# lastz/lastz

Hardware: AMD Instinct MI355X
Metric: Gbp-of-target aligned/sec (whole job, --nogapped HSP path, both strands) (higher is better)
Workload: dtype s32

## Files before the change

lastz_amd/csrc/lz_lut.hpp:

```cpp
#pragma once
#include "lz_common.hpp"

#define LZ_PAD2         128
#define LZ_LUT_ENTRIES  4096
#define LZ_LUT_TOTAL    (2 * LZ_LUT_ENTRIES)
#define LZ_LUT_WIN_G    15
#define LZ_LUT_WIN_B    60
#define LZ_LUT_MAXWIN   3
#define LZ_GRAY(c)      ((c) ^ ((c) >> 1))

struct alignas(8) LzLutEntry { u32 ab; u32 sc; };

struct LzLutParams {
    const u8* t2; const u8* q2;
    const u8* tsp; const u8* qsp;
    const u8* t2x; const u8* tspx;
    const u8* tcode; const u8* qcode;
    s32 xdrop;
};

struct LzLutScan { u32 s; s32 run, best; u32 room, used, alive, nwin; };

#if defined(__HIP_DEVICE_COMPILE__)
LZ_HD u32 lz_alignbit(u32 hi, u32 lo, u32 sh) { return __builtin_amdgcn_alignbit(hi, lo, sh); }
LZ_HD s32 lz_sdot4(u32 a, s32 acc) { return __builtin_amdgcn_sdot4((int)a, 0x01010101, acc, false); }
LZ_HD s32 lz_sdot4m(u32 a, u32 ones, s32 acc) { return __builtin_amdgcn_sdot4((int)a, (int)ones, acc, false); }
LZ_HD u32 lz_byte_pair(u32 hi_src, u32 lo_src, int k)
{ return __builtin_amdgcn_perm(hi_src, lo_src, 0x0C0C0000u | ((u32)(4 + k) << 8) | (u32)k); }
#define LZ_UNROLL_ALL _Pragma("unroll")
#else
LZ_HD u32 lz_alignbit(u32 hi, u32 lo, u32 sh) { sh &= 31u; return sh ? (lo >> sh) | (hi << (32u - sh)) : lo; }
LZ_HD s32 lz_sdot4(u32 a, s32 acc) { for (int k = 0; k < 4; k++) acc += (s32)(int8_t)(a >> (8 * k)); return acc; }
LZ_HD s32 lz_sdot4m(u32 a, u32 ones, s32 acc) { for (int k = 0; k < 4; k++) acc += (s32)(int8_t)(a >> (8 * k)) * (s32)((ones >> (8 * k)) & 0xFFu); return acc; }
LZ_HD u32 lz_byte_pair(u32 hi_src, u32 lo_src, int k) { return (((hi_src >> (8 * k)) & 0xFFu) << 8) | ((lo_src >> (8 * k)) & 0xFFu); }
#define LZ_UNROLL_ALL
#endif
LZ_HD u32 lz_ctz64(u64 x) { return (u32)__builtin_ctzll(x); }
LZ_HD u32 lz_clz64(u64 x) { return (u32)__builtin_clzll(x); }

template <bool SPECIAL> struct LzLutRaw { LzVec16 tv, qv, tm, qm; };
template <> struct LzLutRaw<false> { LzVec16 tv, qv; };
#define LZ_LUT_GBYTE(RIGHT_, g_) ((RIGHT_) ? (g_) : 14 - (g_))
template <bool RIGHT, bool SPECIAL>
LZ_HD void lz_lut_fetch(const LzLutParams& P, u32 s_, s32 diag, LzLutRaw<SPECIAL>& raw)
{
    const u32 st = RIGHT ? s_ + (u32)LZ_PAD2 : s_ - 1u + (u32)LZ_PAD2;
    const u32 sq = st - (u32)diag;
    const u32 back = RIGHT ? 0u : 15u;
    raw.tv = lz_load16(P.t2 + ((st >> 2) - back)); raw.qv = lz_load16(P.q2 + ((sq >> 2) - back));
    if constexpr (SPECIAL) {
        const u32 mback = RIGHT ? 0u : 14u;
        raw.tm = lz_load16(P.tsp + ((st >> 3) - mback)); raw.qm = lz_load16(P.qsp + ((sq >> 3) - mback));
    }
}
template <bool RIGHT>
LZ_HD u64 lz_lut_mask64(const LzVec16& v, s64 s)
{
    if (RIGHT) {
        const u32 k = (u32)((u64)(s + LZ_PAD2) & 7u);
        return ((u64)lz_alignbit(v.w[2], v.w[1], k) << 32) | lz_alignbit(v.w[1], v.w[0], k);
    }
    const u32 k = 17u + (u32)((u64)(s - 1 + LZ_PAD2) & 7u);
    return ((u64)lz_alignbit(v.w[3], v.w[2], k) << 32) | lz_alignbit(v.w[2], v.w[1], k);
}

template <bool RIGHT, bool SPECIAL, bool LIMCHK>
LZ_HD void lz_lut_window(const LzLutParams& P, const LzLutEntry* lut, s32 diag, LzLutScan& st, const LzLutRaw<SPECIAL>& raw, const s32* ctab = nullptr)
{
    const s32 X = P.xdrop;
    const LzLutEntry* const tab = lut + (RIGHT ? 0 : LZ_LUT_ENTRIES);
    const u32 spad = RIGHT ? st.s + (u32)LZ_PAD2 : st.s - 1u + (u32)LZ_PAD2, qpad = spad - (u32)diag;
    u32 tw[4], qw[4];
    {
        const u32 a = RIGHT ? 2u * (spad & 3u) : 2u * (spad & 3u) + 2u;
        const u32 b = RIGHT ? 2u * (qpad & 3u) : 2u * (qpad & 3u) + 2u;
        tw[0] = lz_alignbit(raw.tv.w[1], raw.tv.w[0], a); tw[1] = lz_alignbit(raw.tv.w[2], raw.tv.w[1], a); tw[2] = lz_alignbit(raw.tv.w[3], raw.tv.w[2], a); tw[3] = raw.tv.w[3] >> a;
        qw[0] = lz_alignbit(raw.qv.w[1], raw.qv.w[0], b); qw[1] = lz_alignbit(raw.qv.w[2], raw.qv.w[1], b); qw[2] = lz_alignbit(raw.qv.w[3], raw.qv.w[2], b); qw[3] = raw.qv.w[3] >> b;
    }
    u32 lim = st.room < (u32)LZ_LUT_WIN_B ? st.room : (u32)LZ_LUT_WIN_B;
    bool soft = false;
    if constexpr (SPECIAL) {
        const s64 s = (s64)st.s, sq = s - (s64)diag;
        const u64 sm = lz_lut_mask64<RIGHT>(raw.tm, s) | lz_lut_mask64<RIGHT>(raw.qm, sq);
        const u32 nsp = sm ? (RIGHT ? lz_ctz64(sm) : lz_clz64(sm)) : 64u;
        if (nsp < lim) { soft = true; lim = nsp; }
    }
    u32 xw[4], wc[4];
    LZ_UNROLL_ALL
    for (int k = 0; k < 4; k++) {
        xw[k] = tw[k] ^ qw[k];
        const u32 u = (tw[k] & 0x11111111u) | ((tw[k] >> 1) & 0x22222222u);
        wc[k] = (u | (u >> 2)) & 0x0F0F0F0Fu;
    }
    const u32 glim = lim >> 2;
    s32 run = st.run, m = run - st.best + X;
    u32 np = 0, fsc = 0;
#if !defined(LZ_LUT_NO_EARLY_EXIT) && defined(__HIP_DEVICE_COMPILE__)
    {
#define LZ_LUT_ENTRY_OF(g_) tab[lz_byte_pair(wc[LZ_LUT_GBYTE(RIGHT, g_) >> 2], xw[LZ_LUT_GBYTE(RIGHT, g_) >> 2], LZ_LUT_GBYTE(RIGHT, g_) & 3)]
        LzLutEntry ea = LZ_LUT_ENTRY_OF(0), eb = ea;
        LZ_UNROLL_ALL
        for (int g = 0; g < LZ_LUT_WIN_G; g += 2) {
            if (g + 1 < LZ_LUT_WIN_G) eb = LZ_LUT_ENTRY_OF(g + 1);
            if (m < (s32)(ea.ab & 0xFFFFu)) goto groups_done;
            if (LIMCHK && (u32)g >= glim) goto groups_done;
            { const s32 bq = (s32)ea.ab >> 16; m = lz_sdot4(ea.sc, m < bq ? m : bq); run = lz_sdot4(ea.sc, run); np = (u32)g + 1u; }
            if (g + 1 < LZ_LUT_WIN_G) {
                if (g + 2 < LZ_LUT_WIN_G) ea = LZ_LUT_ENTRY_OF(g + 2);
                if (m < (s32)(eb.ab & 0xFFFFu)) goto groups_done;
                if (LIMCHK && (u32)(g + 1) >= glim) goto groups_done;
                { const s32 bq = (s32)eb.ab >> 16; m = lz_sdot4(eb.sc, m < bq ? m : bq); run = lz_sdot4(eb.sc, run); np = (u32)g + 2u; }
            }
        }
        groups_done:
        fsc = (np & 1u) ? eb.sc : ea.sc;
#undef LZ_LUT_ENTRY_OF
    }
#else
    {
        bool dead = false;
        LZ_UNROLL_ALL
        for (int g = 0; g < LZ_LUT_WIN_G; g++) {
            const int by = LZ_LUT_GBYTE(RIGHT, g);
            const LzLutEntry e = tab[lz_byte_pair(wc[by >> 2], xw[by >> 2], by & 3)];
            if (!dead) fsc = e.sc;
            dead = dead | (m < (s32)(e.ab & 0xFFFFu));
            if (LIMCHK) dead = dead | ((u32)g >= glim);
            const s32 bq = (s32)e.ab >> 16;
            const s32 t = lz_sdot4(e.sc, m < bq ? m : bq);
            const s32 r2 = lz_sdot4(e.sc, run);
            m = dead ? m : t; run = dead ? run : r2; np += dead ? 0u : 1u;
        }
    }
#endif
    u32 r = 0;
    if (np < (u32)LZ_LUT_WIN_G) { r = lim - 4u * np; if (r > 4u) r = 4u; }
    s32 best = run - m + X;
    const u32 sc = fsc;
    bool stop = false; u32 j = 0;
    if (LIMCHK) {
        LZ_UNROLL_ALL
        for (u32 b = 0; b < 4; b++) {
            const bool on = !stop && b < r;
            const s32 nr = run + (s32)(int8_t)(sc >> (8u * b));
            run = on ? nr : run;
            j += on ? 1u : 0u;
            best = (on && nr > best) ? nr : best;
            stop = stop | (on && nr < best - X);
        }
    } else if (r) {
        const s32 p1 = lz_sdot4m(sc, 0x00000001u, m), p2 = lz_sdot4m(sc, 0x00000101u, m), p3 = lz_sdot4m(sc, 0x00010101u, m), p4 = lz_sdot4(sc, m);
        const s32 q2 = p1 | p2, q3 = q2 | p3;
        j = 4u + (u32)(p1 >> 31) + (u32)(q2 >> 31) + (u32)(q3 >> 31);
        stop = (q3 | p4) < 0;
    }
    st.run = run; st.best = best;
    st.used += 4u * np + j;
    st.nwin++;
    if (stop) st.alive = 0;
    else if (r == 4u) st.alive = 2;
    else if (soft) {
        if constexpr (SPECIAL) {
            const u32 p1 = RIGHT ? st.s + lim : st.s - 1u - lim;
            const s32 v = ctab[(LZ_CODE_CLASS(P.tcode[(s64)p1]) << 5) | LZ_CODE_CLASS(P.qcode[(s64)p1 - (s64)diag])];
            st.run += v; st.used += 1u;
            if (st.run > st.best) st.best = st.run;
            const u32 eaten = lim + 1u;
            if (st.run < st.best - X || eaten == st.room) st.alive = 0;
            else { st.alive = 1; st.room -= eaten; st.s = RIGHT ? st.s + eaten : st.s - eaten; }
        }
    }
    else if (lim == st.room) st.alive = 0;
    else { st.alive = 1; st.room -= (u32)LZ_LUT_WIN_B; st.s = RIGHT ? st.s + (u32)LZ_LUT_WIN_B : st.s - (u32)LZ_LUT_WIN_B; }
}
template <bool SPECIAL, bool LIMCHK>
LZ_HD void lz_lut_window_pair(const LzLutParams& P, const LzLutEntry* lut, s32 diag, LzLutScan& L, LzLutScan& R,
                              const LzLutRaw<SPECIAL>& rawl, const LzLutRaw<SPECIAL>& rawr, bool do_l, bool do_r, const s32* ctab = nullptr)
{
    if (do_l) lz_lut_window<false, SPECIAL, LIMCHK>(P, lut, diag, L, rawl, ctab);
    if (do_r) lz_lut_window<true, SPECIAL, LIMCHK>(P, lut, diag, R, rawr, ctab);
}
template <bool RIGHT, bool SPECIAL>
LZ_HD void lz_lut_step(const LzLutParams& P, const LzLutEntry* lut, s32 diag, LzLutScan& st, const s32* ctab = nullptr)
{
    LzLutRaw<SPECIAL> raw;
    lz_lut_fetch<RIGHT, SPECIAL>(P, st.s, diag, raw);
    if (!SPECIAL && st.room >= (u32)LZ_LUT_WIN_B) lz_lut_window<RIGHT, SPECIAL, false>(P, lut, diag, st, raw);
    else                                           lz_lut_window<RIGHT, SPECIAL, true>(P, lut, diag, st, raw, ctab);
}

LZ_HD void lz_lut_init(u64 key, u32 tlen, u32 qlen, s32& diag, LzLutScan& L, LzLutScan& R)
{
    const u32 pos2 = (u32)key;
    diag = (s32)(u32)(key >> 32);
    const u32 pos1 = pos2 + (u32)diag;
    const s32 stopl = diag > 0 ? diag : 0;
    const s32 stopr = ((s32)tlen <= (s32)qlen + diag) ? (s32)tlen : (s32)qlen + diag;
    L.s = R.s = pos1; L.run = L.best = R.run = R.best = 0; L.used = R.used = 0; L.nwin = R.nwin = 0;
    L.room = (u32)((s32)pos1 - stopl); R.room = (u32)(stopr - (s32)pos1);
    L.alive = ((s32)pos1 > stopl) ? 1u : 0u; R.alive = ((s32)pos1 < stopr) ? 1u : 0u;
}

LZ_HD u32 lz_lut_summary(const LzLutScan& L, const LzLutScan& R, s32 min_score)
{
    u32 summ = (L.used & 0xFFu) | ((R.used & 0xFFu) << 8);
    if (L.alive || R.alive || L.best + R.best >= min_score) summ |= LZ_SUMM_SLOW;
    return summ;
}

template <bool SPECIAL>
LZ_HD u32 lz_lut_probe_hit(const LzLutParams& P, const LzLutEntry* lut, u32 tlen, u32 qlen, s32 min_score, u64 key, const s32* ctab = nullptr)
{
    s32 diag; LzLutScan L, R;
    lz_lut_init(key, tlen, qlen, diag, L, R);
    while (L.alive == 1 && L.nwin < (u32)LZ_LUT_MAXWIN) lz_lut_step<false, SPECIAL>(P, lut, diag, L, ctab);
    while (R.alive == 1 && R.nwin < (u32)LZ_LUT_MAXWIN) lz_lut_step<true, SPECIAL>(P, lut, diag, R, ctab);
    return lz_lut_summary(L, R, min_score);
}

LZ_HD u64 lz_hit_record(u64 key, u32 summ)
{
    const u32 pos2 = (u32)key, diag = (u32)(key >> 32);
    const bool slow = (summ & LZ_SUMM_SLOW) != 0;
    const u64 payload = slow ? (u64)(diag >> 16) : (u64)(summ & 0xFFFFu);
    return (u64)pos2 | ((u64)(diag & 0xFFu) << 31) | (payload << 39) | (slow ? (1ull << 63) : 0ull);
}
#define LZ_REC_TAG(r)     ((u32)((r) >> 55) & 0xFFu)
#define LZ_REC_UNTAG(r)   ((r) & ~(0xFFull << 55))
LZ_HD u64 lz_hit_record_tagged(u64 key, u32 summ) { return lz_hit_record(key, summ) | ((u64)((u32)(key >> 40) & 0xFFu) << 55); }

#define LZ_WCTX_BYTES 32
struct alignas(16) LzWctx { u32 w[LZ_WCTX_BYTES / 4]; };
LZ_HD u32 lz_wctx_first_byte(u32 pos1) { return ((pos1 - 1u + (u32)LZ_PAD2) >> 2) - 15u; }
LZ_HD u32 lz_wctx_right_offset(u32 pos1) { return ((pos1 + (u32)LZ_PAD2) >> 2) - lz_wctx_first_byte(pos1); }
LZ_HD LzWctx lz_wctx_make(const u8* two, u32 pos1) { LzWctx e; __builtin_memcpy(&e, two + lz_wctx_first_byte(pos1), LZ_WCTX_BYTES); return e; }
LZ_HD void lz_wctx_windows(const LzWctx& e, u32 pos1, LzVec16& tl, LzVec16& tr)
{
    const bool at16 = lz_wctx_right_offset(pos1) == 16u;
    LZ_UNROLL_ALL
    for (int k = 0; k < 4; k++) {
        tl.w[k] = e.w[k];
        const u32 at15 = lz_alignbit(e.w[4 + k], e.w[3 + k], 24u);
        tr.w[k] = at16 ? e.w[4 + k] : at15;
    }
}

#define LZ_REC_POS2(r)    ((u32)((r) & 0x7FFFFFFFu))
#define LZ_REC_LOW8(r)    ((u32)((r) >> 31) & 0xFFu)
#define LZ_REC_PAYLOAD(r) ((u32)((r) >> 39) & 0xFFFFu)
#define LZ_REC_SLOW(r)    ((u32)((r) >> 63))
LZ_HD u64 lz_rec_with_index(u64 r, u32 idx)
{ return (r & ~((0xFFull << 31) | (0x1Full << 55))) | ((u64)(idx & 0xFFu) << 31) | ((u64)((idx >> 8) & 0x1Fu) << 55); }
#define LZ_REC_INDEX(r)   (((u32)((r) >> 31) & 0xFFu) | (((u32)((r) >> 55) & 0x1Fu) << 8))

template <class Emit>
LZ_HD void lz_settle_record(const LzExtendParams& P, const s32* score_tab, u64 rec, u32 h ,
                            u32& dend, u64& n_ext, u64& n_bp, Emit&& emit)
{
    const u32 p2 = LZ_REC_POS2(rec);
    if (dend > p2 - P.seed_len) return;
    n_ext++;
    const u32 pay = LZ_REC_PAYLOAD(rec);
    if (!LZ_REC_SLOW(rec)) {
        const u32 room = p2 - dend, dlo = pay & 0xFFu, dext = pay >> 8;
        const u32 extent = p2 + dext;
        n_bp += (dlo < room ? dlo : room) + dext;
        if (extent > dend) dend = extent;
        return;
    }
    const s32 diag = (s32)((pay << 16) | h);
    dend = lz_reextend(P, score_tab, p2, diag, dend, n_bp, emit);
}
```

lastz_amd/csrc/scan_kernels.hip:

```cpp
#include <hip/hip_runtime.h>
#include <algorithm>
#include <type_traits>
#include "lz_ctx.hpp"
#include "lz_host.hpp"
#include "lz_lut.hpp"
#include "lz_seed_dev.hpp"

#define LZ_SC_ROUNDS 4

struct LzScanTask { u32 idx; s32 diag; LzLutScan L, R; };
static_assert(sizeof(LzScanTask) == 64, "LzScanTask: one 64-byte line per task");
#define LZ_SC_TPB 512
template <int MODE> struct LzScanShared {
    union {
        LzLutEntry lut[LZ_LUT_TOTAL];
        struct { s32 tab[LZ_NCLASS * LZ_NCLASS]; s32 tab8[64]; } bc;
    };
    s32 ctab[MODE == 1 ? LZ_NCLASS * LZ_NCLASS : 1];
};

template <bool SP>
__device__ __forceinline__ void lz_scan_round(const LzExtendParams& P, const LzLutParams& Q, const LzLutEntry* lut, const s32* ctab, u64 key, bool valid,
                                              const LzLutRaw<SP>& rawl, const LzLutRaw<SP>& rawr, u32 idx, u32 lane,
                                              u32& summ_out, LzScanTask* __restrict__ my_tasks, u32& my_n, u32 region_cap)
{
    constexpr bool HLIM = SP;
    s32 diag; LzLutScan L, R;
    lz_lut_init(key, P.tlen, P.qlen, diag, L, R);
    if (!valid) { L.alive = 0; R.alive = 0; }
    const bool ql = L.alive && !HLIM && L.room < (u32)LZ_LUT_WIN_B, qr = R.alive && !HLIM && R.room < (u32)LZ_LUT_WIN_B;
    lz_lut_window_pair<SP, HLIM>(Q, lut, diag, L, R, rawl, rawr, L.alive && !ql, R.alive && !qr, ctab);
    const bool more = valid && (L.alive == 1 || R.alive == 1);
    const u64 mm = __ballot(more);
    bool queued = false;
    if (mm) {
        const u32 slot = my_n + (u32)__popcll(mm & ((1ull << lane) - 1ull));
        if (more && slot < region_cap) {
            LzScanTask t; t.idx = idx; t.diag = diag; t.L = L; t.R = R;
            my_tasks[slot] = t; queued = true;
        }
        my_n += (u32)__popcll(mm);
    }
    summ_out = queued ? 0u : lz_lut_summary(L, R, P.min_score);
}
template <bool SP>
__device__ __forceinline__ void lz_scan_fetch(const LzLutParams& Q, u64 key, LzLutRaw<SP>& rawl, LzLutRaw<SP>& rawr)
{
    const u32 pos2 = (u32)key, pos1 = pos2 + (u32)(key >> 32);
    const s32 diag = (s32)(u32)(key >> 32);
    const u32 stl = pos1 - 1u + (u32)LZ_PAD2, str = pos1 + (u32)LZ_PAD2;
    const u32 bl = (stl >> 2) - 15u, br = str >> 2;
    const u32 ol = bl + (bl & ~31u);
    rawl.tv = lz_load16(Q.t2x + ol); rawr.tv = lz_load16(Q.t2x + (ol + (br - bl)));
    const u32 sql = stl - (u32)diag, sqr = str - (u32)diag;
    rawl.qv = lz_load16(Q.q2 + ((sql >> 2) - 15u)); rawr.qv = lz_load16(Q.q2 + (sqr >> 2));
    if constexpr (SP) {
        const u32 ml = (stl >> 3) - 14u, mr = str >> 3;
        const u32 oml = ml + (ml & ~31u);
        rawl.tm = lz_load16(Q.tspx + oml); rawr.tm = lz_load16(Q.tspx + (oml + (mr - ml)));
        rawl.qm = lz_load16(Q.qsp + ((sql >> 3) - 14u)); rawr.qm = lz_load16(Q.qsp + (sqr >> 3));
    }
}

template <int MODE, int TPB, int WPE>
__global__ void __launch_bounds__(TPB, WPE)
k_scan_hits(LzExtendParams P, LzLutParams Q, const u64* __restrict__ keys, u64 n,
            const s32* __restrict__ score_tab_g, const LzLutEntry* __restrict__ lut_g,
            u32* __restrict__ summ, u8* __restrict__ bins, LzScanTask* __restrict__ tasks, u32* __restrict__ n_tasks, u32 region_cap)
{
    __shared__ LzScanShared<MODE> sh;
    const u32 tid = threadIdx.x, lane = tid & 63u, w = tid >> 6;
    if (MODE == 1) { for (u32 k = tid; k < LZ_NCLASS * LZ_NCLASS; k += TPB) sh.ctab[k] = score_tab_g[k]; }
    if (MODE < 2) { for (u32 k = tid; k < LZ_LUT_TOTAL; k += TPB) sh.lut[k] = lut_g[k]; }
    else {
        for (u32 k = tid; k < LZ_NCLASS * LZ_NCLASS; k += TPB) sh.bc.tab[k] = score_tab_g[k];
        if (tid < 64) sh.bc.tab8[tid] = score_tab_g[(tid >> 3) * LZ_NCLASS + (tid & 7)];
    }
    __syncthreads();
    const LzLutEntry* lut = sh.lut;
    const s32* const ctab = sh.ctab;
    constexpr bool SP = MODE == 1;
    constexpr u32 SPAN = 64u * LZ_SC_ROUNDS;
    static_assert(LZ_SC_ROUNDS == 4, "the round pipeline below is written out for four rounds per span");
    const u64 nspans = (n + SPAN - 1) / SPAN, wstride = (u64)gridDim.x * (TPB / 64);
    const u32 region = blockIdx.x * (TPB / 64) + w;
    LzScanTask* const my_tasks = tasks + (size_t)region * region_cap;
    u32 my_n = 0;
    u64 span = (u64)blockIdx.x * (TPB / 64) + w;
    if (MODE == 2) {
        for (; span < nspans; span += wstride) {
            const u64 base = span * SPAN;
            const u32 span_n = (n - base < (u64)SPAN) ? (u32)(n - base) : SPAN;
#pragma unroll 1
            for (u32 r = 0; r < LZ_SC_ROUNDS; r++) {
                const u32 li = r * 64u + lane;
                if (li < span_n) { const u64 kk = keys[base + li]; summ[base + li] = lz_probe_hit(P, sh.bc.tab, sh.bc.tab8, P.cls8 != 0, kk); bins[base + li] = (u8)LZ_KEY_BIN(kk); }
            }
        }
    } else if (span < nspans) {
        typedef u64 lz_u64x2 __attribute__((ext_vector_type(2)));
        auto load_keys = [&](u64 sp, u64& a0, u64& a1, u64& a2, u64& a3) {
            const u64 base = sp * SPAN;
            const u32 sn = (n - base < (u64)SPAN) ? (u32)(n - base) : SPAN;
            const u32 l4 = 4u * lane;
            const u64* kp = keys + base + l4;
            if (l4 + 3u < sn) {
                const lz_u64x2 x = LZ_NT_LD(reinterpret_cast<const lz_u64x2*>(kp)), y = LZ_NT_LD(reinterpret_cast<const lz_u64x2*>(kp + 2));
                a0 = x.x; a1 = x.y; a2 = y.x; a3 = y.y;
            } else {
                a0 = (l4 < sn) ? LZ_NT_LD(kp) : 0ull;           a1 = (l4 + 1u < sn) ? LZ_NT_LD(kp + 1) : 0ull;
                a2 = (l4 + 2u < sn) ? LZ_NT_LD(kp + 2) : 0ull;  a3 = 0ull;
            }
        };
        u64 k0, k1, k2, k3;
        load_keys(span, k0, k1, k2, k3);
        LzLutRaw<SP> al, ar, bl, br;
        lz_scan_fetch<SP>(Q, k0, al, ar);
#pragma unroll 1
        for (;;) {
            const u64 base = span * SPAN;
            const u32 span_n = (n - base < (u64)SPAN) ? (u32)(n - base) : SPAN;
            const u32 l4 = 4u * lane;
            const u32 ib = (u32)base + l4;
            const bool more_spans = span + wstride < nspans;
            u64 n0 = 0, n1 = 0, n2 = 0, n3 = 0;
            u32 s0, s1, s2, s3;
            lz_scan_fetch<SP>(Q, k1, bl, br);
            lz_scan_round<SP>(P, Q, lut, ctab, k0, l4 < span_n, al, ar, ib, lane, s0, my_tasks, my_n, region_cap);
            if (more_spans) load_keys(span + wstride, n0, n1, n2, n3);
            lz_scan_fetch<SP>(Q, k2, al, ar);
            lz_scan_round<SP>(P, Q, lut, ctab, k1, l4 + 1u < span_n, bl, br, ib + 1u, lane, s1, my_tasks, my_n, region_cap);
            lz_scan_fetch<SP>(Q, k3, bl, br);
            lz_scan_round<SP>(P, Q, lut, ctab, k2, l4 + 2u < span_n, al, ar, ib + 2u, lane, s2, my_tasks, my_n, region_cap);
            if (more_spans) lz_scan_fetch<SP>(Q, n0, al, ar);
            lz_scan_round<SP>(P, Q, lut, ctab, k3, l4 + 3u < span_n, bl, br, ib + 3u, lane, s3, my_tasks, my_n, region_cap);
            const u32 pbytes = LZ_KEY_BIN(k0) | (LZ_KEY_BIN(k1) << 8) | (LZ_KEY_BIN(k2) << 16) | (LZ_KEY_BIN(k3) << 24);
            if (l4 + 3u < span_n) {
                typedef u32 lz_u32x4 __attribute__((ext_vector_type(4)));
                lz_u32x4 sv4; sv4.x = s0; sv4.y = s1; sv4.z = s2; sv4.w = s3;
                LZ_NT_ST(sv4, reinterpret_cast<lz_u32x4*>(summ + ib));
                LZ_NT_ST(pbytes, reinterpret_cast<u32*>(bins + ib));
            } else {
                if (l4 < span_n)      { summ[ib] = s0;      bins[ib] = (u8)pbytes; }
                if (l4 + 1u < span_n) { summ[ib + 1u] = s1; bins[ib + 1u] = (u8)(pbytes >> 8); }
                if (l4 + 2u < span_n) { summ[ib + 2u] = s2; bins[ib + 2u] = (u8)(pbytes >> 16); }
            }
            if (!more_spans) break;
            span += wstride; k0 = n0; k1 = n1; k2 = n2; k3 = n3;
        }
    }
    if (lane == 0) n_tasks[region] = my_n < region_cap ? my_n : region_cap;
}

#define LZ_ST_TPB 512
template <int MODE, bool TAGGED>
__global__ void __launch_bounds__(LZ_ST_TPB)
k_scan_tasks(LzExtendParams P, LzLutParams Q, const LzLutEntry* __restrict__ lut_g, const s32* __restrict__ score_tab_g, const LzScanTask* __restrict__ tasks,
             const u32* __restrict__ n_tasks, u32 n_regions, u32 region_cap, std::conditional_t<TAGGED, u64, u32>* __restrict__ out)
{
    constexpr bool SP = MODE == 1;
    static_assert(!(SP && TAGGED), "pos1 is recovered from the windows a scan ran: without special bytes only");
    __shared__ LzLutEntry lut[LZ_LUT_TOTAL];
    __shared__ s32 ctab[SP ? LZ_NCLASS * LZ_NCLASS : 1];
    for (u32 k = threadIdx.x; k < LZ_LUT_TOTAL; k += LZ_ST_TPB) lut[k] = lut_g[k];
    if (SP) for (u32 k = threadIdx.x; k < LZ_NCLASS * LZ_NCLASS; k += LZ_ST_TPB) ctab[k] = score_tab_g[k];
    __syncthreads();
    for (u32 region = blockIdx.x; region < n_regions; region += gridDim.x) {
        const u32 nt = n_tasks[region];
        for (u32 k = threadIdx.x; k < nt; k += (u32)LZ_ST_TPB) {
            const LzScanTask t = tasks[(size_t)region * region_cap + k];
            LzLutScan L = t.L, R = t.R;
            u32 pos1 = 0;
            if constexpr (TAGGED) pos1 = L.alive == 1 ? L.s + (u32)LZ_LUT_WIN_B * L.nwin : R.s - (u32)LZ_LUT_WIN_B * R.nwin;
            while (L.alive == 1 && L.nwin < (u32)LZ_LUT_MAXWIN) lz_lut_step<false, SP>(Q, lut, t.diag, L, ctab);
            while (R.alive == 1 && R.nwin < (u32)LZ_LUT_MAXWIN) lz_lut_step<true, SP>(Q, lut, t.diag, R, ctab);
            const u32 summ = lz_lut_summary(L, R, P.min_score);
            if constexpr (TAGGED) out[t.idx] = lz_hit_record_tagged(lz_hit_key(pos1, pos1 - (u32)t.diag), summ);
            else                  LZ_NT_ST(summ, out + t.idx);
        }
    }
}

static int lz_scan_tpb(int mode)
{
    return mode != 0 ? LZ_SC_TPB : 640;
}
static int lz_task_regions(LzCtx& c, int mode, u64 n, u32 n_regions, u32& region_cap)
{
    region_cap = (u32)std::min<u64>(n / (mode == 1 ? 12 : 32) / n_regions + 64, 1u << 20);
    if (const u32 force = lz_settings().task_region_cap) region_cap = force;
    int rc;
    if (mode < 2 && (rc = c.scan_tasks.ensure((size_t)n_regions * region_cap * sizeof(LzScanTask)))) return rc;
    return c.scan_ntasks.ensure((size_t)n_regions * 4);
}
static int lz_scan_buffers(LzCtx& c, int mode, u64 n, u32& grid, u32& n_regions, u32& region_cap)
{
    const u32 wpg = (u32)lz_scan_tpb(mode) / 64u;
    const int cus = c.num_cus;
    const u64 nspans = (n + 64u * LZ_SC_ROUNDS - 1) / (64u * LZ_SC_ROUNDS), want = (nspans + wpg - 1) / wpg;
    grid = (u32)std::min<u64>(want ? want : 1, 2u * (u64)cus);
    n_regions = grid * wpg;
    const int rc = c.summ.ensure((size_t)n * 4);
    return rc ? rc : lz_task_regions(c, mode, n, n_regions, region_cap);
}
int lzk_scan_reserve(LzCtx& c, int mode, u64 max_n)
{
    u32 grid, n_regions, region_cap;
    return lz_scan_buffers(c, mode, max_n, grid, n_regions, region_cap);
}

int lzk_scan_hits(LzCtx& c, int mode, const LzExtendParams& P, const LzLutParams& Q, u64 n)
{
    if (n == 0) return 0;
    const int cus = c.num_cus;
    int rc;
    u32 grid, n_regions, task_cap;
    if ((rc = lz_scan_buffers(c, mode, n, grid, n_regions, task_cap))) return rc;
    const u64* keys = c.keys.as<u64>(); const s32* score_tab = c.score_tab.as<s32>(); const LzLutEntry* lut = c.lut.as<LzLutEntry>();
    u32* summ = c.summ.as<u32>(); u8* bins = c.bins.as<u8>(); LzScanTask* tasks = c.scan_tasks.as<LzScanTask>(); u32* ntk = c.scan_ntasks.as<u32>();
    c.timer.begin("k_scan_hits", c.stream);
#define LZ_SCAN_LAUNCH(M_, T_, W_) hipLaunchKernelGGL((k_scan_hits<M_, T_, W_>), dim3(grid), dim3(T_), 0, c.stream, P, Q, keys, n, score_tab, lut, summ, bins, tasks, ntk, task_cap)
    if (mode == 0)      LZ_SCAN_LAUNCH(0, 640, 5);
    else if (mode == 1) LZ_SCAN_LAUNCH(1, LZ_SC_TPB, 4);
    else                LZ_SCAN_LAUNCH(2, LZ_SC_TPB, 4);
#undef LZ_SCAN_LAUNCH
    c.timer.end(c.stream);
    LZ_HIP(hipGetLastError());
    if (mode < 2) {
        const dim3 tgrid(std::min<u32>(n_regions, 4u * (u32)cus));
        c.timer.begin("k_scan_tasks", c.stream);
        if (mode == 0) hipLaunchKernelGGL((k_scan_tasks<0, false>), tgrid, dim3(LZ_ST_TPB), 0, c.stream, P, Q, lut, score_tab, tasks, ntk, n_regions, task_cap, summ);
        else           hipLaunchKernelGGL((k_scan_tasks<1, false>), tgrid, dim3(LZ_ST_TPB), 0, c.stream, P, Q, lut, score_tab, tasks, ntk, n_regions, task_cap, summ);
        c.timer.end(c.stream);
        LZ_HIP(hipGetLastError());
    }
    return 0;
}

struct LzFuseTrip { u32 p1, pos2, dst; bool ok; LzWctx cx; LzVec16 ql, qr; };

template <bool SELF, int TPB, int CAP>
__global__ void __launch_bounds__(TPB)
k_scan_hits2(u32 lo, u32 i0, u32 i1, LzSeedDev sd,
             const u32* __restrict__ wstart, const u32* __restrict__ wpos, const LzWctx* __restrict__ wctx,
             const u32* __restrict__ sk, const u32* __restrict__ sv, u32 n, const u64* __restrict__ off, u64 base,
             LzExtendParams P, LzLutParams Q, const LzLutEntry* __restrict__ lut_g,
             u64* __restrict__ recs, LzScanTask* __restrict__ tasks, u32* __restrict__ n_tasks, u32 region_cap, LzSelfDev self)
{
    __shared__ LzLutEntry lut[LZ_LUT_TOTAL];
    constexpr int WORDS = CAP / 2 / 64;
    __shared__ LzListWave<CAP> shw[TPB / 64];
    for (u32 k = threadIdx.x; k < LZ_LUT_TOTAL; k += TPB) lut[k] = lut_g[k];
    __syncthreads();
    LzListWave<CAP>& sh = shw[threadIdx.x >> 6];
    unsigned short* const own = reinterpret_cast<unsigned short*>(sh.own32);
    const u32 lane = threadIdx.x & 63u;
    const u32 region = blockIdx.x * (TPB / 64) + (threadIdx.x >> 6), nwaves = gridDim.x * (TPB / 64);
    LzScanTask* const my_tasks = tasks + (size_t)region * region_cap;
    u32 my_n = 0;
    const u32 ngroups = (n + 63u) / 64u;
    for (u32 grp = region; grp < ngroups; grp += nwaves) {
        const u32 j = grp * 64u + lane;
        u32 w_l = 0, i_l = 0; bool in = false;
        if (j < n) { w_l = sk[j] & ((2u << sd.weight) - 1u); i_l = sv[j]; in = !(w_l >> sd.weight) && i_l >= i0 && i_l < i1; }
        if (!__ballot(in)) continue;
        const u32 dbase = in ? (u32)(off[i_l] - base) : 0u;
        const u32 pos2 = lo + i_l + 1u;
        u32 slo = 0, shi = 0;
        if (SELF) lz_self_bounds(self, pos2, slo, shi);
        u32 carry = 0;
        for (int r = 0; r < sd.nprobes; r += LZ_FILL_GROUP) {
            u32 la[LZ_FILL_GROUP], len[LZ_FILL_GROUP]; u32 total = 0;
#pragma unroll
            for (int p = 0; p < LZ_FILL_GROUP; p++) {
                const bool on = in && r + p < sd.nprobes;
                const u32 w = on ? (w_l ^ sd.probe_xor[(r + p) & (LZ_MAX_PROBES - 1)]) : 0u;
                la[p] = wstart[w]; len[p] = wstart[w + 1];
            }
#pragma unroll
            for (int p = 0; p < LZ_FILL_GROUP; p++) {
                const bool on = in && r + p < sd.nprobes;
                len[p] = on ? len[p] - la[p] : 0u;
                if (!SELF) total += len[p];
            }
            if (SELF) {
                lz_clip_runs<LZ_FILL_GROUP>(wpos, la, len, slo, shi);
#pragma unroll
                for (int p = 0; p < LZ_FILL_GROUP; p++) total += len[p];
            }
            u32 inc = total;
            LZ_WAVE_SCAN_U32(inc, total, lz_uadd)
            const u32 E = inc - total;
            const u32 T = (u32)__builtin_amdgcn_readlane((int)inc, 63);
            {
                u32 S = E;
#pragma unroll
                for (int p = 0; p < LZ_FILL_GROUP; p++) { sh.lsrc[lane * LZ_FILL_GROUP + p] = la[p] - S; S += len[p]; }
            }
            sh.ent[lane] = make_uint2(dbase + carry - E, pos2);
            for (u32 cs = 0; cs < T; cs += CAP) {
                const u32 tc = (T - cs < (u32)CAP) ? T - cs : (u32)CAP;
                uint4* const mine = reinterpret_cast<uint4*>(sh.own32 + lane * WORDS);
#pragma unroll
                for (int k = 0; k < WORDS / 4; k++) mine[k] = make_uint4(0u, 0u, 0u, 0u);
                __atomic_signal_fence(__ATOMIC_SEQ_CST);
                {
                    u32 S = E;
#pragma unroll
                    for (int p = 0; p < LZ_FILL_GROUP; p++) {
                        const u32 l = len[p];
                        if (l && S < cs + tc && S + l > cs) own[(S > cs ? S : cs) - cs] = (unsigned short)(1u + lane * LZ_FILL_GROUP + (u32)p);
                        S += l;
                    }
                }
                __atomic_signal_fence(__ATOMIC_SEQ_CST);
                u32 wv[WORDS];
#pragma unroll
                for (int k = 0; k < WORDS / 4; k++) { const uint4 v = mine[k]; wv[4 * k] = v.x; wv[4 * k + 1] = v.y; wv[4 * k + 2] = v.z; wv[4 * k + 3] = v.w; }
                u32 segmax = 0;
#pragma unroll
                for (int k = 0; k < WORDS; k++) { const u32 m2 = lz_umax(wv[k] & 0xFFFFu, wv[k] >> 16); segmax = lz_umax(segmax, m2); }
                u32 sinc = segmax;
                LZ_WAVE_SCAN_U32(sinc, segmax, lz_umax)
                u32 run = lz_dpp_u32<0x138, 0xf, 0xf>(0u, sinc);
#pragma unroll
                for (int k = 0; k < WORDS; k++) {
                    const u32 a0 = lz_umax(wv[k] & 0xFFFFu, run), a1 = lz_umax(wv[k] >> 16, a0);
                    wv[k] = a0 | (a1 << 16); run = a1;
                }
#pragma unroll
                for (int k = 0; k < WORDS / 4; k++) mine[k] = make_uint4(wv[4 * k], wv[4 * k + 1], wv[4 * k + 2], wv[4 * k + 3]);
                __atomic_signal_fence(__ATOMIC_SEQ_CST);
                auto load_trip = [&](u32 tb, LzFuseTrip& t) {
                    const u32 t0 = tb + lane;
                    t.ok = t0 < tc;
                    const u32 tt = t.ok ? t0 : tc - 1u;
                    const u32 list = (u32)own[tt] - 1u;
                    const u32 ls = sh.lsrc[list];
                    const uint2 en = sh.ent[list / LZ_FILL_GROUP];
                    const u32 tabs = cs + tt, e = ls + tabs;
                    t.p1 = wpos[e]; t.cx = wctx[e];
                    t.pos2 = en.y; t.dst = en.x + tabs;
                    const u32 sql = en.y - 1u + (u32)LZ_PAD2;
                    t.ql = lz_load16(Q.q2 + ((sql >> 2) - 15u)); t.qr = lz_load16(Q.q2 + ((sql + 1u) >> 2));
                };
                auto scan_trip = [&](const LzFuseTrip& t) {
                    const u64 key = lz_hit_key(t.p1, t.pos2);
                    LzLutRaw<false> rl, rr;
                    lz_wctx_windows(t.cx, t.p1, rl.tv, rr.tv);
                    rl.qv = t.ql; rr.qv = t.qr;
                    u32 summ;
                    lz_scan_round<false>(P, Q, lut, nullptr, key, t.ok, rl, rr, t.dst, lane, summ, my_tasks, my_n, region_cap);
                    if (t.ok) LZ_NT_ST(lz_hit_record_tagged(key, summ), recs + t.dst);
                };
                LzFuseTrip ta, tb2;
                load_trip(0u, ta);
#pragma unroll 1
                for (u32 tb = 0;;) {
                    if (tb + 64u < tc) load_trip(tb + 64u, tb2);
                    scan_trip(ta);
                    tb += 64u; if (tb >= tc) break;
                    if (tb + 64u < tc) load_trip(tb + 64u, ta);
                    scan_trip(tb2);
                    tb += 64u; if (tb >= tc) break;
                }
                __atomic_signal_fence(__ATOMIC_SEQ_CST);
            }
            carry += total;
        }
    }
    if (lane == 0) n_tasks[region] = my_n < region_cap ? my_n : region_cap;
}

static u32 lz_fused_tpb(LzCtx& c)
{
    return c.self.mode != LZ_SELF_OFF ? 512u : 1024u;
}
static int lz_fused_buffers(LzCtx& c, u64 n_hits, u32& grid, u32& n_regions, u32& region_cap)
{
    const int cus = c.num_cus;
    grid = (u32)cus; n_regions = grid * (lz_fused_tpb(c) / 64u);
    return lz_task_regions(c, 0, n_hits, n_regions, region_cap);
}
int lzk_fused_reserve(LzCtx& c, u64 max_n)
{
    u32 grid, n_regions, region_cap;
    return lz_fused_buffers(c, max_n, grid, n_regions, region_cap);
}
int lzk_scan_fused(LzCtx& c, u32 lo, const LzChunk& ch, u32 n, const LzExtendParams& P, const LzLutParams& Q)
{
    if (n == 0 || ch.i1 <= ch.i0 || ch.nh == 0) return 0;
    const u32* sk = c.wsk.as<u32>(); const u32* sv = c.wsv.as<u32>();
    lz_chunk_range(c, ch.i0, ch.i1, sk, sv, n);
    if (n == 0) return 0;
    int rc;
    u32 grid, n_regions, region_cap;
    if ((rc = lz_fused_buffers(c, ch.nh, grid, n_regions, region_cap))) return rc;
    const LzLutEntry* lut = c.lut.as<LzLutEntry>(); u64* tagged = c.keys.as<u64>();
    LzScanTask* tasks = c.scan_tasks.as<LzScanTask>(); u32* ntk = c.scan_ntasks.as<u32>();
    c.timer.begin("k_scan_hits", c.stream);
#define LZ_FUSED_LAUNCH(S_, T_, C_, self_) hipLaunchKernelGGL((k_scan_hits2<S_, T_, C_>), dim3(grid), dim3(T_), 0, c.stream, lo, ch.i0, ch.i1, c.seed, c.wstart.as<u32>(), c.wpos.as<u32>(), \
                           c.wctx.as<LzWctx>(), sk, sv, n, c.off.as<u64>(), ch.base, P, Q, lut, tagged, tasks, ntk, region_cap, self_)
    if (c.self.mode != LZ_SELF_OFF) LZ_FUSED_LAUNCH(true, 512, 2560, c.self);
    else                            LZ_FUSED_LAUNCH(false, 1024, 512, LzSelfDev{});
#undef LZ_FUSED_LAUNCH
    c.timer.end(c.stream);
    LZ_HIP(hipGetLastError());
    c.timer.begin("k_scan_tasks", c.stream);
    hipLaunchKernelGGL((k_scan_tasks<0, true>), dim3(std::min<u32>(n_regions, 4u * grid)), dim3(LZ_ST_TPB), 0, c.stream, P, Q, lut, (const s32*)nullptr, tasks, ntk, n_regions, region_cap, tagged);
    c.timer.end(c.stream);
    LZ_HIP(hipGetLastError());
    return 0;
}
```

lastz_amd/csrc/table_kernels.hip:

```cpp
#include <hip/hip_runtime.h>
#include <rocprim/device/device_radix_sort.hpp>
#include "lz_ctx.hpp"
#include "lz_lut.hpp"
#include "lz_seed_dev.hpp"

__global__ void __launch_bounds__(LZ_TPB)
k_table_words(const u8* __restrict__ tcode, u32 start, u32 end, u32 step, LzSeedDev sd,
              u32* __restrict__ keys, u32* __restrict__ vals, u32 n)
{
    u32 j = blockIdx.x * LZ_TPB + threadIdx.x;
    if (j >= n) return;
    u32 p = end - j;
    u32 key = 1u << sd.weight;
    if (p >= start + (u32)sd.length && (p % step) == 0) {
        u32 packed;
        if (lz_window_word(tcode, p, sd, packed)) key = packed;
    }
    keys[j] = key; vals[j] = p;
}

__global__ void __launch_bounds__(LZ_TPB)
k_key_bounds_u32(const u32* __restrict__ keys, u32 n, u32 nwords, u32* __restrict__ wstart)
{
    u32 i = blockIdx.x * LZ_TPB + threadIdx.x;
    if (i > n) return;
    s64 kp = (i == 0) ? -1 : (s64)keys[i - 1];
    s64 k  = (i == n) ? (s64)nwords : (s64)keys[i];
    if (k > (s64)nwords) k = nwords;
    if (kp > (s64)nwords) kp = nwords;
    for (s64 w = kp + 1; w <= k; w++) wstart[w] = i;
}

int lzk_table_build(LzCtx& c)
{
    const lz_table_geom& g = c.geom;
    const u32 n = g.end - g.start;
    const u32 nwords = 1u << c.seed.weight;
    int rc;
    if ((rc = c.tb_keys.ensure((size_t)n * 4))) return rc;
    if ((rc = c.tb_vals.ensure((size_t)n * 4))) return rc;
    if ((rc = c.tb_keys2.ensure((size_t)n * 4))) return rc;
    if ((rc = c.tb_vals2.ensure((size_t)n * 4))) return rc;
    if ((rc = c.wstart.ensure(((size_t)nwords + 1) * 4))) return rc;

    c.timer.begin("k_table_words", c.stream);
    hipLaunchKernelGGL(k_table_words, dim3((n + LZ_TPB - 1) / LZ_TPB), dim3(LZ_TPB), 0, c.stream,
                       c.target.code_base(), g.start, g.end, g.step, c.seed,
                       c.tb_keys.as<u32>(), c.tb_vals.as<u32>(), n);
    c.timer.end(c.stream);
    LZ_HIP(hipGetLastError());

    size_t tmp = 0;
    LZ_HIP(rocprim::radix_sort_pairs(nullptr, tmp, c.tb_keys.as<u32>(), c.tb_keys2.as<u32>(),
                                     c.tb_vals.as<u32>(), c.tb_vals2.as<u32>(), (size_t)n, 0u,
                                     (unsigned)c.seed.weight + 1u, c.stream));
    if ((rc = c.sort_tmp.ensure(tmp))) return rc;
    c.timer.begin("rocprim_sort_table", c.stream);
    LZ_HIP(rocprim::radix_sort_pairs(c.sort_tmp.p, tmp, c.tb_keys.as<u32>(), c.tb_keys2.as<u32>(),
                                     c.tb_vals.as<u32>(), c.tb_vals2.as<u32>(), (size_t)n, 0u,
                                     (unsigned)c.seed.weight + 1u, c.stream));
    c.timer.end(c.stream);

    c.timer.begin("k_key_bounds_u32", c.stream);
    hipLaunchKernelGGL(k_key_bounds_u32, dim3((n + 1 + LZ_TPB - 1) / LZ_TPB), dim3(LZ_TPB), 0, c.stream,
                       c.tb_keys2.as<u32>(), n, nwords, c.wstart.as<u32>());
    c.timer.end(c.stream);
    LZ_HIP(hipGetLastError());

    u32 nw = 0;
    LZ_HIP(hipMemcpyAsync(&nw, c.wstart.as<u32>() + nwords, 4, hipMemcpyDeviceToHost, c.stream));
    LZ_HIP(hipStreamSynchronize(c.stream));
    c.timer.resolve();
    c.num_words = nw;
    c.table_gen++;
    if ((rc = c.wpos.ensure((size_t)(nw ? nw : 1) * 4))) return rc;
    LZ_HIP(hipMemcpyAsync(c.wpos.p, c.tb_vals2.p, (size_t)nw * 4, hipMemcpyDeviceToDevice, c.stream));
    LZ_HIP(hipStreamSynchronize(c.stream));
    return 0;
}

__global__ void __launch_bounds__(LZ_TPB)
k_table_export(const u32* __restrict__ wstart, const u32* __restrict__ wpos, u32 nwords,
               u32 adj_start, u32 step, u32* __restrict__ last, u32* __restrict__ prev)
{
    u32 w = blockIdx.x * LZ_TPB + threadIdx.x;
    if (w >= nwords) return;
    u32 a = wstart[w], b = wstart[w + 1];
    if (a == b) return;
    if (last) last[w] = (wpos[a] - adj_start) / step;
    if (prev)
        for (u32 j = a; j < b; j++)
            prev[(wpos[j] - adj_start) / step] = (j + 1 < b) ? (wpos[j + 1] - adj_start) / step : 0xFFFFFFFFu;
}

int lzk_table_export(LzCtx& c, u32* last_dev, u32* prev_dev, u32 prev_entries)
{
    const u32 nwords = 1u << c.seed.weight;
    if (last_dev) LZ_HIP(hipMemsetAsync(last_dev, 0, (size_t)nwords * 4, c.stream));
    if (prev_dev) LZ_HIP(hipMemsetAsync(prev_dev, 0, (size_t)prev_entries * 4, c.stream));
    u32 adj = c.geom.start - (c.geom.start % c.geom.step);
    hipLaunchKernelGGL(k_table_export, dim3((nwords + LZ_TPB - 1) / LZ_TPB), dim3(LZ_TPB), 0, c.stream,
                       c.wstart.as<u32>(), c.wpos.as<u32>(), nwords, adj, c.geom.step, last_dev, prev_dev);
    LZ_HIP(hipGetLastError());
    return 0;
}

__global__ void __launch_bounds__(LZ_TPB)
k_build_wctx(const u32* __restrict__ wpos, u64 num_words, const u8* __restrict__ two, LzVec16* __restrict__ wctx)
{
    const u64 j = (u64)blockIdx.x * LZ_TPB + threadIdx.x;
    if (j >= 2 * num_words) return;
    const u32 pos1 = wpos[j >> 1];
    wctx[j] = lz_load16(two + lz_wctx_first_byte(pos1) + 16u * (u32)(j & 1u));
}

int lzk_wctx_build(LzCtx& c)
{
    const u64 nw = c.num_words;
    if (nw == 0) return 0;
    c.timer.begin("k_build_wctx", c.stream);
    hipLaunchKernelGGL(k_build_wctx, dim3((unsigned)((2 * nw + LZ_TPB - 1) / LZ_TPB)), dim3(LZ_TPB), 0, c.stream,
                       c.wpos.as<u32>(), nw, c.target.two.as<u8>(), c.wctx.as<LzVec16>());
    c.timer.end(c.stream);
    LZ_HIP(hipGetLastError());
    return 0;
}
```

Measured before the change: 0.4075.

## Pre-align target word context at table build and parameterize LUT prefetch depth

The word-context table now stores target windows already shifted into alignment for the left and right scans, so the fused scan path can skip the per-hit alignbit shifts on the target side. A DEPTH template parameter is added to the LUT window walk, generalising the two-entry prefetch into a ring of DEPTH entries. Compile-time macros select the depth per call site, and all of them default to 2. The build kernel now loads the right window from a position-dependent offset and aligns it, which changes the layout that the fused consumer assumes.

```diff
diff --git a/lastz_amd/csrc/lz_lut.hpp b/lastz_amd/csrc/lz_lut.hpp
--- a/lastz_amd/csrc/lz_lut.hpp
+++ b/lastz_amd/csrc/lz_lut.hpp
@@ -64,7 +64,7 @@
     return ((u64)lz_alignbit(v.w[3], v.w[2], k) << 32) | lz_alignbit(v.w[2], v.w[1], k);
 }
 
-template <bool RIGHT, bool SPECIAL, bool LIMCHK>
+template <bool RIGHT, bool SPECIAL, bool LIMCHK, int DEPTH = 2, bool TALIGNED = false>
 LZ_HD void lz_lut_window(const LzLutParams& P, const LzLutEntry* lut, s32 diag, LzLutScan& st, const LzLutRaw<SPECIAL>& raw, const s32* ctab = nullptr)
 {
     const s32 X = P.xdrop;
@@ -74,7 +74,8 @@
     {
         const u32 a = RIGHT ? 2u * (spad & 3u) : 2u * (spad & 3u) + 2u;
         const u32 b = RIGHT ? 2u * (qpad & 3u) : 2u * (qpad & 3u) + 2u;
-        tw[0] = lz_alignbit(raw.tv.w[1], raw.tv.w[0], a); tw[1] = lz_alignbit(raw.tv.w[2], raw.tv.w[1], a); tw[2] = lz_alignbit(raw.tv.w[3], raw.tv.w[2], a); tw[3] = raw.tv.w[3] >> a;
+        if constexpr (TALIGNED) { tw[0] = raw.tv.w[0]; tw[1] = raw.tv.w[1]; tw[2] = raw.tv.w[2]; tw[3] = raw.tv.w[3]; }
+        else { tw[0] = lz_alignbit(raw.tv.w[1], raw.tv.w[0], a); tw[1] = lz_alignbit(raw.tv.w[2], raw.tv.w[1], a); tw[2] = lz_alignbit(raw.tv.w[3], raw.tv.w[2], a); tw[3] = raw.tv.w[3] >> a; }
         qw[0] = lz_alignbit(raw.qv.w[1], raw.qv.w[0], b); qw[1] = lz_alignbit(raw.qv.w[2], raw.qv.w[1], b); qw[2] = lz_alignbit(raw.qv.w[3], raw.qv.w[2], b); qw[3] = raw.qv.w[3] >> b;
     }
     u32 lim = st.room < (u32)LZ_LUT_WIN_B ? st.room : (u32)LZ_LUT_WIN_B;
@@ -96,8 +97,8 @@
     s32 run = st.run, m = run - st.best + X;
     u32 np = 0, fsc = 0;
 #if !defined(LZ_LUT_NO_EARLY_EXIT) && defined(__HIP_DEVICE_COMPILE__)
-    {
 #define LZ_LUT_ENTRY_OF(g_) tab[lz_byte_pair(wc[LZ_LUT_GBYTE(RIGHT, g_) >> 2], xw[LZ_LUT_GBYTE(RIGHT, g_) >> 2], LZ_LUT_GBYTE(RIGHT, g_) & 3)]
+    if constexpr (DEPTH == 2) {
         LzLutEntry ea = LZ_LUT_ENTRY_OF(0), eb = ea;
         LZ_UNROLL_ALL
         for (int g = 0; g < LZ_LUT_WIN_G; g += 2) {
@@ -114,8 +115,26 @@
         }
         groups_done:
         fsc = (np & 1u) ? eb.sc : ea.sc;
+    } else {
+        LzLutEntry e[DEPTH];
+        e[0] = LZ_LUT_ENTRY_OF(0);
+        LZ_UNROLL_ALL
+        for (int k = 1; k < DEPTH; k++) e[k] = (k < DEPTH - 1) ? LZ_LUT_ENTRY_OF(k) : e[0];
+        LZ_UNROLL_ALL
+        for (int g = 0; g < LZ_LUT_WIN_G; g++) {
+            if (g + DEPTH - 1 < LZ_LUT_WIN_G) e[(g + DEPTH - 1) % DEPTH] = LZ_LUT_ENTRY_OF(g + DEPTH - 1);
+            const LzLutEntry eg = e[g % DEPTH];
+            if (m < (s32)(eg.ab & 0xFFFFu)) goto groups_done_n;
+            if (LIMCHK && (u32)g >= glim) goto groups_done_n;
+            { const s32 bq = (s32)eg.ab >> 16; m = lz_sdot4(eg.sc, m < bq ? m : bq); run = lz_sdot4(eg.sc, run); np = (u32)g + 1u; }
+        }
+        groups_done_n:
+        const u32 k = np % (u32)DEPTH;
+        fsc = e[0].sc;
+        LZ_UNROLL_ALL
+        for (int d = 1; d < DEPTH; d++) fsc = (k == (u32)d) ? e[d].sc : fsc;
+    }
 #undef LZ_LUT_ENTRY_OF
-    }
 #else
     {
         bool dead = false;
@@ -173,20 +192,20 @@
     else if (lim == st.room) st.alive = 0;
     else { st.alive = 1; st.room -= (u32)LZ_LUT_WIN_B; st.s = RIGHT ? st.s + (u32)LZ_LUT_WIN_B : st.s - (u32)LZ_LUT_WIN_B; }
 }
-template <bool SPECIAL, bool LIMCHK>
+template <bool SPECIAL, bool LIMCHK, int DEPTH = 2, bool TALIGNED = false>
 LZ_HD void lz_lut_window_pair(const LzLutParams& P, const LzLutEntry* lut, s32 diag, LzLutScan& L, LzLutScan& R,
                               const LzLutRaw<SPECIAL>& rawl, const LzLutRaw<SPECIAL>& rawr, bool do_l, bool do_r, const s32* ctab = nullptr)
 {
-    if (do_l) lz_lut_window<false, SPECIAL, LIMCHK>(P, lut, diag, L, rawl, ctab);
-    if (do_r) lz_lut_window<true, SPECIAL, LIMCHK>(P, lut, diag, R, rawr, ctab);
-}
-template <bool RIGHT, bool SPECIAL>
+    if (do_l) lz_lut_window<false, SPECIAL, LIMCHK, DEPTH, TALIGNED>(P, lut, diag, L, rawl, ctab);
+    if (do_r) lz_lut_window<true, SPECIAL, LIMCHK, DEPTH, TALIGNED>(P, lut, diag, R, rawr, ctab);
+}
+template <bool RIGHT, bool SPECIAL, int DEPTH = 2>
 LZ_HD void lz_lut_step(const LzLutParams& P, const LzLutEntry* lut, s32 diag, LzLutScan& st, const s32* ctab = nullptr)
 {
     LzLutRaw<SPECIAL> raw;
     lz_lut_fetch<RIGHT, SPECIAL>(P, st.s, diag, raw);
-    if (!SPECIAL && st.room >= (u32)LZ_LUT_WIN_B) lz_lut_window<RIGHT, SPECIAL, false>(P, lut, diag, st, raw);
-    else                                           lz_lut_window<RIGHT, SPECIAL, true>(P, lut, diag, st, raw, ctab);
+    if (!SPECIAL && st.room >= (u32)LZ_LUT_WIN_B) lz_lut_window<RIGHT, SPECIAL, false, DEPTH>(P, lut, diag, st, raw);
+    else                                           lz_lut_window<RIGHT, SPECIAL, true, DEPTH>(P, lut, diag, st, raw, ctab);
 }
 
 LZ_HD void lz_lut_init(u64 key, u32 tlen, u32 qlen, s32& diag, LzLutScan& L, LzLutScan& R)
@@ -243,6 +262,28 @@
         const u32 at15 = lz_alignbit(e.w[4 + k], e.w[3 + k], 24u);
         tr.w[k] = at16 ? e.w[4 + k] : at15;
     }
+}
+LZ_HD u32 lz_wctx_shift(u32 pos1, bool right) { return right ? 2u * ((pos1 + (u32)LZ_PAD2) & 3u) : 2u * ((pos1 - 1u + (u32)LZ_PAD2) & 3u) + 2u; }
+LZ_HD LzVec16 lz_wctx_align(const LzVec16& v, u32 sh)
+{
+    LzVec16 t;
+    t.w[0] = lz_alignbit(v.w[1], v.w[0], sh); t.w[1] = lz_alignbit(v.w[2], v.w[1], sh); t.w[2] = lz_alignbit(v.w[3], v.w[2], sh); t.w[3] = v.w[3] >> sh;
+    return t;
+}
+LZ_HD LzWctx lz_wctx_make_aligned(const u8* two, u32 pos1)
+{
+    LzVec16 tl, tr;
+    lz_wctx_windows(lz_wctx_make(two, pos1), pos1, tl, tr);
+    const LzVec16 al = lz_wctx_align(tl, lz_wctx_shift(pos1, false)), ar = lz_wctx_align(tr, lz_wctx_shift(pos1, true));
+    LzWctx e;
+    LZ_UNROLL_ALL
+    for (int k = 0; k < 4; k++) { e.w[k] = al.w[k]; e.w[4 + k] = ar.w[k]; }
+    return e;
+}
+LZ_HD void lz_wctx_aligned_windows(const LzWctx& e, LzVec16& tl, LzVec16& tr)
+{
+    LZ_UNROLL_ALL
+    for (int k = 0; k < 4; k++) { tl.w[k] = e.w[k]; tr.w[k] = e.w[4 + k]; }
 }
 
 #define LZ_REC_POS2(r)    ((u32)((r) & 0x7FFFFFFFu))
diff --git a/lastz_amd/csrc/scan_kernels.hip b/lastz_amd/csrc/scan_kernels.hip
--- a/lastz_amd/csrc/scan_kernels.hip
+++ b/lastz_amd/csrc/scan_kernels.hip
@@ -6,6 +6,18 @@
 #include "lz_lut.hpp"
 #include "lz_seed_dev.hpp"
 
+#ifndef LZ_DEPTH_FUSED
+#define LZ_DEPTH_FUSED 2
+#endif
+#ifndef LZ_DEPTH_FUSED_SELF
+#define LZ_DEPTH_FUSED_SELF 2
+#endif
+#ifndef LZ_DEPTH_SPLIT
+#define LZ_DEPTH_SPLIT 2
+#endif
+#ifndef LZ_DEPTH_TASKS
+#define LZ_DEPTH_TASKS 2
+#endif
 #define LZ_SC_ROUNDS 4
 
 struct LzScanTask { u32 idx; s32 diag; LzLutScan L, R; };
@@ -19,7 +31,7 @@
     s32 ctab[MODE == 1 ? LZ_NCLASS * LZ_NCLASS : 1];
 };
 
-template <bool SP>
+template <bool SP, int DEPTH, bool TALIGNED = false>
 __device__ __forceinline__ void lz_scan_round(const LzExtendParams& P, const LzLutParams& Q, const LzLutEntry* lut, const s32* ctab, u64 key, bool valid,
                                               const LzLutRaw<SP>& rawl, const LzLutRaw<SP>& rawr, u32 idx, u32 lane,
                                               u32& summ_out, LzScanTask* __restrict__ my_tasks, u32& my_n, u32 region_cap)
@@ -29,7 +41,7 @@
     lz_lut_init(key, P.tlen, P.qlen, diag, L, R);
     if (!valid) { L.alive = 0; R.alive = 0; }
     const bool ql = L.alive && !HLIM && L.room < (u32)LZ_LUT_WIN_B, qr = R.alive && !HLIM && R.room < (u32)LZ_LUT_WIN_B;
-    lz_lut_window_pair<SP, HLIM>(Q, lut, diag, L, R, rawl, rawr, L.alive && !ql, R.alive && !qr, ctab);
+    lz_lut_window_pair<SP, HLIM, DEPTH, TALIGNED>(Q, lut, diag, L, R, rawl, rawr, L.alive && !ql, R.alive && !qr, ctab);
     const bool more = valid && (L.alive == 1 || R.alive == 1);
     const u64 mm = __ballot(more);
     bool queued = false;
@@ -126,14 +138,14 @@
             u64 n0 = 0, n1 = 0, n2 = 0, n3 = 0;
             u32 s0, s1, s2, s3;
             lz_scan_fetch<SP>(Q, k1, bl, br);
-            lz_scan_round<SP>(P, Q, lut, ctab, k0, l4 < span_n, al, ar, ib, lane, s0, my_tasks, my_n, region_cap);
+            lz_scan_round<SP, LZ_DEPTH_SPLIT>(P, Q, lut, ctab, k0, l4 < span_n, al, ar, ib, lane, s0, my_tasks, my_n, region_cap);
             if (more_spans) load_keys(span + wstride, n0, n1, n2, n3);
             lz_scan_fetch<SP>(Q, k2, al, ar);
-            lz_scan_round<SP>(P, Q, lut, ctab, k1, l4 + 1u < span_n, bl, br, ib + 1u, lane, s1, my_tasks, my_n, region_cap);
+            lz_scan_round<SP, LZ_DEPTH_SPLIT>(P, Q, lut, ctab, k1, l4 + 1u < span_n, bl, br, ib + 1u, lane, s1, my_tasks, my_n, region_cap);
             lz_scan_fetch<SP>(Q, k3, bl, br);
-            lz_scan_round<SP>(P, Q, lut, ctab, k2, l4 + 2u < span_n, al, ar, ib + 2u, lane, s2, my_tasks, my_n, region_cap);
+            lz_scan_round<SP, LZ_DEPTH_SPLIT>(P, Q, lut, ctab, k2, l4 + 2u < span_n, al, ar, ib + 2u, lane, s2, my_tasks, my_n, region_cap);
             if (more_spans) lz_scan_fetch<SP>(Q, n0, al, ar);
-            lz_scan_round<SP>(P, Q, lut, ctab, k3, l4 + 3u < span_n, bl, br, ib + 3u, lane, s3, my_tasks, my_n, region_cap);
+            lz_scan_round<SP, LZ_DEPTH_SPLIT>(P, Q, lut, ctab, k3, l4 + 3u < span_n, bl, br, ib + 3u, lane, s3, my_tasks, my_n, region_cap);
             const u32 pbytes = LZ_KEY_BIN(k0) | (LZ_KEY_BIN(k1) << 8) | (LZ_KEY_BIN(k2) << 16) | (LZ_KEY_BIN(k3) << 24);
             if (l4 + 3u < span_n) {
                 typedef u32 lz_u32x4 __attribute__((ext_vector_type(4)));
@@ -172,8 +184,8 @@
             LzLutScan L = t.L, R = t.R;
             u32 pos1 = 0;
             if constexpr (TAGGED) pos1 = L.alive == 1 ? L.s + (u32)LZ_LUT_WIN_B * L.nwin : R.s - (u32)LZ_LUT_WIN_B * R.nwin;
-            while (L.alive == 1 && L.nwin < (u32)LZ_LUT_MAXWIN) lz_lut_step<false, SP>(Q, lut, t.diag, L, ctab);
-            while (R.alive == 1 && R.nwin < (u32)LZ_LUT_MAXWIN) lz_lut_step<true, SP>(Q, lut, t.diag, R, ctab);
+            while (L.alive == 1 && L.nwin < (u32)LZ_LUT_MAXWIN) lz_lut_step<false, SP, LZ_DEPTH_TASKS>(Q, lut, t.diag, L, ctab);
+            while (R.alive == 1 && R.nwin < (u32)LZ_LUT_MAXWIN) lz_lut_step<true, SP, LZ_DEPTH_TASKS>(Q, lut, t.diag, R, ctab);
             const u32 summ = lz_lut_summary(L, R, P.min_score);
             if constexpr (TAGGED) out[t.idx] = lz_hit_record_tagged(lz_hit_key(pos1, pos1 - (u32)t.diag), summ);
             else                  LZ_NT_ST(summ, out + t.idx);
@@ -347,10 +359,10 @@
                 auto scan_trip = [&](const LzFuseTrip& t) {
                     const u64 key = lz_hit_key(t.p1, t.pos2);
                     LzLutRaw<false> rl, rr;
-                    lz_wctx_windows(t.cx, t.p1, rl.tv, rr.tv);
+                    lz_wctx_aligned_windows(t.cx, rl.tv, rr.tv);
                     rl.qv = t.ql; rr.qv = t.qr;
                     u32 summ;
-                    lz_scan_round<false>(P, Q, lut, nullptr, key, t.ok, rl, rr, t.dst, lane, summ, my_tasks, my_n, region_cap);
+                    lz_scan_round<false, SELF ? LZ_DEPTH_FUSED_SELF : LZ_DEPTH_FUSED, true>(P, Q, lut, nullptr, key, t.ok, rl, rr, t.dst, lane, summ, my_tasks, my_n, region_cap);
                     if (t.ok) LZ_NT_ST(lz_hit_record_tagged(key, summ), recs + t.dst);
                 };
                 LzFuseTrip ta, tb2;
diff --git a/lastz_amd/csrc/table_kernels.hip b/lastz_amd/csrc/table_kernels.hip
--- a/lastz_amd/csrc/table_kernels.hip
+++ b/lastz_amd/csrc/table_kernels.hip
@@ -111,7 +111,8 @@
     const u64 j = (u64)blockIdx.x * LZ_TPB + threadIdx.x;
     if (j >= 2 * num_words) return;
     const u32 pos1 = wpos[j >> 1];
-    wctx[j] = lz_load16(two + lz_wctx_first_byte(pos1) + 16u * (u32)(j & 1u));
+    const bool right = (j & 1u) != 0;
+    wctx[j] = lz_wctx_align(lz_load16(two + lz_wctx_first_byte(pos1) + (right ? lz_wctx_right_offset(pos1) : 0u)), lz_wctx_shift(pos1, right));
 }
 
 int lzk_wctx_build(LzCtx& c)
```

After: 0.4164 (median of 6 runs). 2.2% higher.
